# awkrail/svpc

Hardware: AMD Instinct MI355X
Metric: train steps/sec (vivt, batch=16, clip_seq=12) (higher is better)
Workload: dtype bf16x3; 1 GPU; MODEL_TYPE=vivt train step: N=16 videos/GPU x S=12 clips x Lv=100 frames x F=3072, Lt=22, D=768, H=12, L=6 (enc+step-enc+dec), V=951, A=384, E=10; dropout .1/.1/.4; fwd+bwd+allreduce+clip+BertAdam; mode=bf16x3, global_batch=16, parallelism=dp1, launch=hipGraph replay, gpus_requested=1

## Files before the change

include/svpc_hip.h:

```cpp
#ifndef SVPC_HIP_H
#define SVPC_HIP_H
#include <stddef.h>
#ifdef __cplusplus
extern "C" {
#endif

typedef struct ihipStream_t* svpc_stream_t;
typedef unsigned long long svpc_u64;

#define SVPC_ACT_NONE 0
#define SVPC_ACT_RELU 1
#define SVPC_ACT_GELU 2
#define SVPC_ACT_SIGMOID 3

const char* svpc_last_error(void);
int svpc_abi_version(void);

int svpc_ln_fwd(const float* x, const int* src_rows, const float* res, const float* gamma, const float* beta, float* y,
                float* mean, float* rstd, int R, int D, float eps, float p_pre, unsigned site_pre, float p_post,
                unsigned site_post, const svpc_u64* seed, const float* add1, int mod1, const float* add2, const int* idx2,
                svpc_stream_t stream);
int svpc_ln_fwd_t(const void* x, int x_dt, const int* src_rows, const void* res, const float* gamma, const float* beta, void* y,
                  int y_dt, float* mean, float* rstd, int R, int D, float eps, float p_pre, unsigned site_pre, float p_post,
                  unsigned site_post, const svpc_u64* seed, const float* add1, int mod1, const float* add2, const int* idx2,
// ... 196 lines not shown
                             svpc_stream_t stream);
int svpc_ptr_attn_gate_bwd_r(const float* dec, const float* proj, const float* bank, const int* step_ne, const float* pi, const float* dpi,
                             const float* pgen, const float* dpgen, const float* pgen_w, float* ddec, float* dproj, float* dbank,
                             float* wpart, int T, int lt, int e_max, int D, const int* row_off, const int* row_len, svpc_stream_t stream);
int svpc_ptr_mix_loss_fwd(const float* logits, const float* g, const float* pi, const int* labels, const int* row_c,
                          const int* row_vid, const int* csr_off, const int* csr_ent, const int* csr_id, const float* csr_w, float* P,
                          float* loss_rows, int R, int V, int c_max, int e_max, float smoothing, svpc_stream_t stream);
int svpc_ptr_mix_loss_bwd(const float* logits, const float* g, const float* pi, const int* labels, const int* row_c,
                          const int* row_vid, const int* csr_off, const int* csr_ent, const int* csr_id, const float* csr_w,
                          const float* P, const float* dP_ext, const float* dloss, float* dlogits, float* dg, float* dpi, int R, int V,
                          int c_max, int e_max, float smoothing, svpc_stream_t stream);
int svpc_ce_row_weights(const int* labels, const int* row_vid, int R, int n_vid, float* row_w, svpc_stream_t stream);
int svpc_ptr_mix_ce_fwd(const float* logits, const float* g, const float* pi, const int* labels, const int* row_c,
                        const int* row_vid, const int* csr_off, const int* csr_ent, const int* csr_id, const float* csr_w, float* P,
                        float* loss_rows, int R, int V, int c_max, int e_max, float smoothing, const float* row_w, svpc_stream_t stream);
int svpc_ptr_mix_ce_bwd(const float* logits, const float* g, const float* pi, const int* labels, const int* row_c,
                        const int* row_vid, const int* csr_off, const int* csr_ent, const int* csr_id, const float* csr_w,
                        const float* P, const float* dP_ext, const float* dloss, float* dlogits, float* dg, float* dpi, int R, int V,
                        int c_max, int e_max, float smoothing, const float* row_w, svpc_stream_t stream);

int svpc_gumbel_noise(float* out, size_t n, unsigned site, const svpc_u64* seed, svpc_stream_t stream);
int svpc_gumbel_fwd(const float* P, const float* noise, const int* row_c, const float* emb, float* bow, int* idx, float* stats, int R,
                    int c_max, int V, int W, float tau, svpc_stream_t stream);
int svpc_gumbel_bwd(const float* P, const float* noise, const int* row_c, const float* stats, const float* dy, float* dP, int R,
                    int c_max, int V, float tau, svpc_stream_t stream);
int svpc_gumbel_emb_grad(const float* dbow, const int* idx, const float* stats, float* demb, int R, int V, int W,
                         svpc_stream_t stream);

int svpc_rownorm_fwd(const float* a, float* y, int R, int C, int mode, svpc_stream_t stream);
int svpc_rownorm_bwd(const float* dy, const float* y, const float* a, float* da, int R, int C, int mode, svpc_stream_t stream);
int svpc_span_mean_fwd(const float* x, const int* starts, const int* lens, const float* w, const float* add, const int* add_idx,
                       float* out, int G, int D, svpc_stream_t stream);
int svpc_span_mean_bwd(const float* dout, const int* starts, const int* lens, const float* w, float* dx, int G, int D,
                       svpc_stream_t stream);
int svpc_scatter_add_rows(const float* dx, const int* idx, float* dtable, int R, int D, int pad_row, svpc_stream_t stream);
int svpc_bce_rows_fwd(const float* p, const float* y, const int* widths, float* out, int R, int C, svpc_stream_t stream);
int svpc_bce_rows_bwd(const float* dout, const float* p, const float* y, const int* widths, float* dp, int R, int C,
                      svpc_stream_t stream);
int svpc_asl_rows_fwd(const float* p, const float* y, const float* active, float* out, int R, int C, float gneg, float gpos,
                      float clip, float eps, svpc_stream_t stream);
int svpc_asl_rows_bwd(const float* dout, const float* p, const float* y, const float* active, float* dp, int R, int C, float gneg,
                      float gpos, float clip, float eps, svpc_stream_t stream);
int svpc_loss_tail_ws_floats(int n_cap, int R);
int svpc_loss_tail_fwd(const float* cap_rows, int n_cap, const float* e_p, const float* align, const int* widths, int R, int Ce,
                       const float* a_p, const float* act, int Ca, const float* r_e, const float* r_a, float lambda, float gneg,
                       float gpos, float clip, float eps, float* out5, float* workspace, int* counter, svpc_stream_t stream);
int svpc_loss_tail_bwd(const float* dout, int n_cap, const float* e_p, const float* align, const int* widths, int R, int Ce,
                       const float* a_p, const float* act, int Ca, const float* r_e, const float* r_a, float lambda, float gneg,
                       float gpos, float clip, float eps, float* d_cap, float* de_p, float* da_p, float* dr_e, float* dr_a,
                       svpc_stream_t stream);
int svpc_row_any_eq1(const float* x, float* out, int R, int C, svpc_stream_t stream);
int svpc_gather_cast_multi(const void* segments, int n, svpc_stream_t stream);
int svpc_gather_cast_multi_seed(const void* segments, int n, svpc_u64* bump_seed, svpc_stream_t stream);
int svpc_clamp_labels(const int* in, int* out, int n, int vocab, int unk, svpc_stream_t stream);
int svpc_lstm_cell_fwd(const float* gx, const float* gh, const float* c_prev, const float* h_prev, const float* active, float* h,
                       float* c, float* gates_act, int N, int D, svpc_stream_t stream);
int svpc_lstm_cell_bwd(const float* dh, const float* dc, const float* gates_act, const float* c_prev, const float* active,
                       float* dgates, float* dc_prev, float* dh_prev, int N, int D, svpc_stream_t stream);
int svpc_metric_argmax(const float* scores, int ld, int R, int C, const long long* labels, int ignore, double* counters,
                       svpc_stream_t stream);
int svpc_metric_f1(const float* prob, const float* gold, size_t n, double* counters, svpc_stream_t stream);
int svpc_gather_rows_f32(const float* src, const int* idx, float* dst, int rows, int width, svpc_stream_t stream);
int svpc_video_tokens(const int* n_valid, long long* ids, float* mask, int clips, int Lv, int L, int cls_id, int vid_id, int sep_id,
                      int pad_id, svpc_stream_t stream);
int svpc_lstm_cell_fwd_idx(const float* gx_all, const int* rows, const float* gh, const float* c_prev, const float* h_prev,
                           const float* active, float* h, float* c, float* gates_act, int N, int D, svpc_stream_t stream);
int svpc_lstm_cell_bwd_seq(const float* dh_out, const float* dh_rec, const float* dc, const float* gates_act, const float* c_prev,
                           const float* active, float* dgates, float* dc_prev, float* dh_prev, int N, int D, svpc_stream_t stream);
int svpc_lstm_pair_fwd(const float* const* gx, const int* const* rows, const float* const* gh, const float* const* c_prev,
                       const float* const* h_prev, const float* active, float* const* h, float* const* c, float* const* gates, int N, int D,
                       svpc_stream_t stream);
int svpc_lstm_pair_step_fwd(const float* const* h_prev, const float* const* c_prev, const float* const* w_hh, const float* const* gx,
                            const int* const* rows, const float* active, float* const* h, float* const* c, float* const* gates, int N,
                            int D, svpc_stream_t stream);
int svpc_lstm_pair_step_fwd_x3(const float* const* h_prev, const float* const* c_prev, const float* const* w_hh, const float* const* gx,
                               const int* const* rows, const float* active, float* const* h, float* const* c, float* const* gates, int N,
                               int D, svpc_stream_t stream);
int svpc_lstm_pair_bwd(const float* const* dh_out, const float* const* dh_rec, const float* const* dc, const float* const* gates,
                       const float* const* c_prev, const float* active, float* const* dgates, float* const* dc_prev,
                       float* const* dh_prev, int N, int D, svpc_stream_t stream);
int svpc_lstm_pair_bwd_parts(const float* const* dh_out, const float* const* dh_rec, const float* const* dh_parts, int n_parts,
                             const float* const* dc, const float* const* gates, const float* const* c_prev, const float* active,
                             float* const* dgates, float* const* dc_prev, float* const* dh_prev, int N, int D, svpc_stream_t stream);
int svpc_greedy_pick(const float* scores, int ld, const int* row_c, const int* row_x, int n_sent, int lt, int pos, int unk,
                     int* next_ext, int* next_model, svpc_stream_t stream);
int svpc_greedy_pick_append(const float* scores, int ld, const int* row_c, const int* row_x, int n_sent, int lt, int pos, int unk,
                            int* next_ext, int* next_model, int* text_out, int* ext_out, int ld_out, int col, svpc_stream_t stream);
int svpc_beam_step(const float* scores, int ld, const int* row_c, const int* row_x, int n_sent, int beam, int pos, int logits, int unk,
                   int eos, int pad, int slot_rows, float* cum, int* finished, const int* text_in, const int* ext_in, const int* rows_in,
                   int* text_out, int* ext_out, int* rows_out, int ld_tok, int* parent, int* next_ext, int* next_model, svpc_stream_t stream);
int svpc_beam_finalize(const float* cum, const int* ext, int ld_tok, int n_sent, int beam, int lt, int* best_ids, float* best_score,
                       svpc_stream_t stream);
int svpc_beam_step_ctl(const float* scores, int ld, const int* row_c, const int* row_x, int n_sent, int beam, int pos, int logits, int unk,
                       int eos, int pad, int slot_rows, float* cum, int* finished, const int* text_in, const int* ext_in, const int* rows_in,
                       int* text_out, int* ext_out, int* rows_out, int ld_tok, int* parent, int* next_ext, int* next_model, int min_len,
                       int ngram, const unsigned* excl, int excl_v, const double* lp, int* len, svpc_stream_t stream);
int svpc_beam_step_para(const float* scores, int ld, const int* row_c, const int* row_x, int n_sent, int beam, int pos, int logits, int unk,
                        int eos, int pad, int slot_rows, float* cum, int* finished, const int* text_in, const int* ext_in, const int* rows_in,
                        int* text_out, int* ext_out, int* rows_out, int ld_tok, int* parent, int* next_ext, int* next_model, int min_len,
                        int ngram, const unsigned* excl, int excl_v, const double* lp, int* len, const int* hist, const int* hist_desc,
                        int bos, svpc_stream_t stream);
int svpc_beam_step_groups(const float* scores, int ld, const int* row_c, const int* row_x, int n_sent, int beam, int pos, int logits, int unk,
                          int eos, int pad, int slot_rows, float* cum, int* finished, const int* text_in, const int* ext_in, const int* rows_in,
                          int* text_out, int* ext_out, int* rows_out, int ld_tok, int* parent, int* next_ext, int* next_model, int min_len,
                          int ngram, const unsigned* excl, int excl_v, const double* lp, int* len, int groups, const float* pen, float* aug,
                          svpc_stream_t stream);
int svpc_beam_finalize_nbest(const float* cum, const int* len, const double* lp, const int* ext, int ld_tok, int n_sent, int beam, int lt,
                             int n_best, int* best_ids, float* best_score, int* best_len, svpc_stream_t stream);
int svpc_sample_step(const float* scores, int ld, const int* row_c, const int* row_x, int n_rows, int max_c, int pos, int logits, int unk,
                     int eos, int pad, double temp, int topk, double topp, int min_len, const long long* seed, float* cum, int* finished,
                     int* len, int* text_out, int* ext_out, int ld_tok, int* next_ext, int* next_model, svpc_stream_t stream);
int svpc_sample_seed(const long long* src, long long* word, long long* used, svpc_stream_t stream);
int svpc_caption_clean(const void* ids, int ids64, long long ld, int row_stride, int row_pick, int n_rows, int lt, long long pad,
                       long long eos, long long ignore, int remove_dup, int* words, int* len, svpc_stream_t stream);
int svpc_caption_ngram_counts(const int* words, const int* len, const int* vid_off, int n_vid, int lt, int period, int comma, int vocab,
                              int* counts, unsigned* vocab_bits, svpc_stream_t stream);
int svpc_decode_metric_accum(const int* counts, int n_vid, double* acc, svpc_stream_t stream);
int svpc_caption_ingredients(const int* words, const int* len, int n_rows, int lt, const int* vid_off, const int* row_vs, int n_vid,
                             const unsigned* pred, int pred_ld, int n_pred, const unsigned* a_bits, int vocab, const int* vid,
                             const int* ing_tok, const int* tok_row, const unsigned* tok_oov, const int* eq_ids, const unsigned* oov_a,
                             const unsigned* gt_mask, const int* gt_len, const int* gx_off, const int* gx_ids, long long* masks, int* extra,
                             int* row_counts, int* vid_counts, unsigned long long* acc, svpc_stream_t stream);
int svpc_caption_tokens(const int* words, const int* len, const int* vid_off, int n_vid, int lt, int vocab, const int* voc_off,
                        const int* voc_tok, int n_voc_tok, const int* vid, const int* oov_off, int n_oov_off, const int* oov_tok,
                        int n_oov_tok, int* tokens, int* tok_len, svpc_stream_t stream);
int svpc_caption_score_counts(const int* tokens, const int* tok_len, int n_vid, const int* vid, const double* ref_norm,
                              const unsigned short* ref_tok, long long n_ref_tok, const unsigned long long* tab_key, const double* tab_idf,
                              int tab_cap, double log_docs, const double* gauss, int* counts, double* scores, long long* seen, int n_seen,
                              svpc_stream_t stream);
int svpc_caption_score_accum(const int* counts, const double* scores, int n_vid, unsigned long long* acc_i, double* acc_f,
                             svpc_stream_t stream);
int svpc_consensus_tokens(const int* words, const int* len, long long n_rows, const int* streams, int n_streams, int lt, int vocab,
                          const int* voc_off, const int* voc_tok, int n_voc_tok, const int* vid, int n_vid, const int* oov_off, int n_oov_off,
                          const int* oov_tok, int n_oov_tok, unsigned short* tokens, int* tok_len, svpc_stream_t stream);
int svpc_consensus_pair_scores(const unsigned short* tokens, const int* tok_len, int n_grp, int k, const unsigned long long* tab_key,
                               const double* tab_idf, int tab_cap, double log_docs, const double* gauss, double* out, double* work,
                               svpc_stream_t stream);
int svpc_consensus_pick(const double* pair, int n_grp, int k, int col, int posterior, const float* scores, const int* grp_off,
                        long long n_rows, const void* ids, int ids64, int lt, const long long* lengths, int* pick, double* expected,
                        long long* out_ids, long long* row_pick, float* out_scores, long long* out_len, svpc_stream_t stream);

int svpc_force_inputs(const void* ids, int ids_i64, int n_cap, int lt, int vocab, int unk, int eos, int pad, int ignore, int* model_ids,
                      float* mask, int* tgt, int* len, int* finished, svpc_stream_t stream);
int svpc_force_score(const float* scores, int ld, const int* row_c, int max_c, const int* tgt, const int* len, int n_cap, int lt, int logits,
                     int unk, int skip, float* step, int* rank, int* top, float* top_step, svpc_stream_t stream);
int svpc_force_finish(const int* tgt, const int* len, const int* row_c, int n_cap, int lt, int unk, int skip, float* step, int* rank,
                      int* top, float* top_step, float* cum, int* n_scored, svpc_stream_t stream);
int svpc_force_accum(const float* cum, const int* n_scored, const int* finished, const int* len, const int* rank, int n_cap, int lt,
                     double* acc, svpc_stream_t stream);

int svpc_seq_nll_fwd(const float* scores, int ld, const int* row_c, int max_c, const int* tgt, const int* len, const float* row_w,
                     int n_cap, int lt, int logits, int unk, float* step, float* cum, int* barred, float* loss, svpc_stream_t stream);
int svpc_seq_nll_bwd(const float* scores, int ld, const int* row_c, int max_c, const int* tgt, const int* len, const int* barred,
                     const float* row_w, const float* dl, int n_cap, int lt, int logits, int unk, float* dscores, int ld_out,
                     svpc_stream_t stream);
int svpc_scst_weights(const double* reward, const double* greedy, const int* row_vid, int n_vid, int k, int n_sent, int rule,
                      double* advantage, float* w, svpc_stream_t stream);

int svpc_rows_move(const void* src, int src_kind, int ld_src, int lo_src, const int* idx, void* dst, int dst_kind, int ld_dst, int lo_dst,
                   int R, int W, svpc_stream_t stream);
int svpc_scatter_add_rows_bf16(const float* rows, const int* idx, void* table, int ld_table, int R, int W, svpc_stream_t stream);
int svpc_pair_rows(float* a, const int* ia, float* b, const int* ib, float* out, float* out2, int R, int W, int mode, svpc_stream_t stream);
int svpc_add_cast_bf16(const void* a, const float* b, void* out, size_t n, svpc_stream_t stream);
int svpc_rows_expand(const float* src, const int* inv, float* out, int n_rows, int W, svpc_stream_t stream);
int svpc_add(const float* a, const float* b, float* c, size_t n, svpc_stream_t stream);
int svpc_sum_all(const float* x, size_t n, float* out, float scale, svpc_stream_t stream);
// ... 16 lines not shown
```

svpc_amd/csrc/gemm_l32.hip:

```cpp
#include "gemm_common.h"
#include <stdlib.h>

typedef __bf16 bf16x8 __attribute__((ext_vector_type(8)));
typedef const void __attribute__((address_space(1))) * l32_gptr;
typedef void __attribute__((address_space(3))) * l32_lptr;

constexpr int L32_BK = 32;
__device__ __attribute__((aligned(16))) const float l32_zeros[4] = {0.f, 0.f, 0.f, 0.f};

template <int N> __device__ __forceinline__ void l32_wait_vmcnt() { asm volatile("s_waitcnt vmcnt(%0)" ::"n"(N) : "memory"); }

template <int R, bool KC>
__device__ __forceinline__ const float* l32_src(const float* P, int ld, int m0, int rows, int k0, int j, int lane) {
    if (KC) {
        const int row = 8 * j + (lane >> 3), pos = lane & 7;
        const int c = pos ^ ((row >> 1) & 7);
        const int gr = min(m0 + row, rows - 1);
        return P + (size_t)gr * ld + k0 + 4 * c;
    } else {
        constexpr int CPR = R / 4;
        const int krow = j * (64 / CPR) + lane / CPR, c = lane % CPR;
        const int gm = min(m0 + 4 * c, rows - 4);
        return P + (size_t)(k0 + krow) * ld + gm;
    }
// ... 486 lines not shown
    skinny_partials<B_KC, NW, X3>(part, arow, brow, ldb, K);
    const u64 seed = epi.p_drop > 0.f ? epi.seed[0] : 0ull;
    const float inv_keep = epi.p_drop > 0.f ? 1.0f / (1.0f - epi.p_drop) : 1.0f;
    const int col = threadIdx.x & 31;
    constexpr int NE = 16 / NW;
    float vs[NE]; int rs[NE], cs[NE]; bool oks[NE];
#pragma unroll
    for (int i = 0; i < NE; ++i) {
        const int row = (threadIdx.x >> 5) + 2 * NW * i;
        const int e = (row & 3) + 4 * (row >> 3), l = col + 32 * ((row >> 2) & 1);
        float v = part[0][e][l];
#pragma unroll
        for (int w = 1; w < NW; ++w) v += part[w][e][l];
        vs[i] = v;
        oks[i] = row < ts && col < ts && m0 + row < M && n0 + col < N;
        rs[i] = min(m0 + row, M - 1); cs[i] = min(n0 + col, N - 1);
    }
    epilogue_store_n<NE>(vs, rs, cs, oks, C, ldc, epi, seed, inv_keep);
}
template <bool B_KC, bool X3 = false>
__global__ __launch_bounds__(256) void gemm_skinny_kernel(const float* __restrict__ A, int lda, const float* __restrict__ B, int ldb,
                                                          float* __restrict__ C, int ldc, int M, int N, int K, Epi epi, int tiles_n, int ts) {
    __shared__ float part[4][16][64];
    const int tm = blockIdx.x / tiles_n, tn = blockIdx.x - tm * tiles_n;
    skinny_tile<B_KC, 4, X3>(part, A, lda, B, ldb, C, ldc, M, N, K, epi, tm, tn, ts);
}
template <int NW, bool X3 = false, bool B_KC = true>
__global__ __launch_bounds__(64 * NW) void gemm_group_skinny_kernel(GemmGroupArgs g) {
    __shared__ float part[NW][16][64];
    int pi = 0;
    while (pi + 1 < g.n && (int)blockIdx.x >= g.p[pi + 1].tile0) ++pi;
    const GemmProb& q = g.p[pi];
    const int tile = blockIdx.x - q.tile0;
    const int tm = tile / q.tiles_n, tn = tile - tm * q.tiles_n;
    Epi epi{nullptr, ACT_NONE, 0.f, 0u, nullptr, g.accumulate, nullptr};
    skinny_tile<B_KC, NW, X3>(part, q.A, q.lda, q.B, q.ldb, q.C, q.ldc, q.M, q.N, q.K, epi, tm, tn);
}

struct LstmStep {
    const float* h_prev[2]; const float* c_prev[2]; const float* w_hh[2]; const float* gx[2]; const int* rows[2]; const float* active;
    float* h[2]; float* c[2]; float* gates[2]; int N, D;
};
template <bool X3>
__global__ __launch_bounds__(256) void lstm_pair_step_fwd_kernel(LstmStep a) {
    __shared__ float part[4][16][64];
    const int z = blockIdx.y, u0 = blockIdx.x * 8, m0 = blockIdx.z * 32;
    const int lane = threadIdx.x & 63, r = lane & 31, hh = lane >> 5;
    const int N = a.N, D = a.D;
    const float* arow = a.h_prev[z] + (size_t)min(m0 + r, N - 1) * D + 8 * hh;
    const float* brow = a.w_hh[z] + (size_t)((r >> 3) * D + u0 + (r & 7)) * D + 8 * hh;
    const int row = threadIdx.x >> 3, j = threadIdx.x & 7, n = m0 + row;
    const int nc = min(n, N - 1), dpre = u0 + j;
    const float* gxp = a.gx[z] + (size_t)a.rows[z][nc] * 4 * D + dpre;
    const float gx0 = gxp[0], gx1 = gxp[D], gx2 = gxp[2 * D], gx3 = gxp[3 * D];
    const float cp_pre = a.c_prev[z][(size_t)nc * D + dpre], hp_pre = a.h_prev[z][(size_t)nc * D + dpre], act_pre = a.active[nc];
    skinny_partials<true, 4, X3>(part, arow, brow, D, D);
    if (n >= N) return;
    float gsum[4];
    const int e = (row & 3) + 4 * (row >> 3), lb = 32 * ((row >> 2) & 1);
#pragma unroll
    for (int g = 0; g < 4; ++g) {
        const int l = g * 8 + j + lb;
        float v = part[0][e][l];
#pragma unroll
        for (int w = 1; w < 4; ++w) v += part[w][e][l];
        gsum[g] = v;
    }
    const int d = u0 + j;
    const size_t i = (size_t)n * D + d, g0 = (size_t)n * 4 * D + d;
    const float gi = sigmoidf_(gx0 + gsum[0]);
    const float gf = sigmoidf_(gx1 + gsum[1]);
    const float gg = tanhf(gx2 + gsum[2]);
    const float go = sigmoidf_(gx3 + gsum[3]);
    float* ga = a.gates[z];
    ga[g0] = gi; ga[g0 + D] = gf; ga[g0 + 2 * D] = gg; ga[g0 + 3 * D] = go;
    const float cp = cp_pre;
    const float cn = gf * cp + gi * gg;
    const float hn = go * tanhf(cn);
    const float act = act_pre;
    a.c[z][i] = act * cn + (1.f - act) * cp;
    a.h[z][i] = act * hn + (1.f - act) * hp_pre;
}

extern "C" {

static int lstm_pair_step_fwd_x(const float* const* h_prev, const float* const* c_prev, const float* const* w_hh, const float* const* gx,
                                const int* const* rows, const float* active, float* const* h, float* const* c, float* const* gates, int N,
                                int D, int x3, hipStream_t stream) {
    if (N == 0) return 0;
    SVPC_REQUIRE(D % 16 == 0 && D >= 16, "lstm_pair_step_fwd: hidden size must be a multiple of 16");
    LstmStep a{};
    for (int z = 0; z < 2; ++z) {
        SVPC_REQUIRE(((((uintptr_t)h_prev[z]) | ((uintptr_t)w_hh[z])) & 15) == 0, "lstm_pair_step_fwd: 16-byte aligned state / weight rows");
        a.h_prev[z] = h_prev[z]; a.c_prev[z] = c_prev[z]; a.w_hh[z] = w_hh[z]; a.gx[z] = gx[z]; a.rows[z] = rows[z];
        a.h[z] = h[z]; a.c[z] = c[z]; a.gates[z] = gates[z];
    }
    a.active = active; a.N = N; a.D = D;
    if (x3) hipLaunchKernelGGL(lstm_pair_step_fwd_kernel<true>, dim3(D / 8, 2, ceil_div(N, 32)), dim3(256), 0, stream, a);
    else hipLaunchKernelGGL(lstm_pair_step_fwd_kernel<false>, dim3(D / 8, 2, ceil_div(N, 32)), dim3(256), 0, stream, a);
    return svpc_check_launch("lstm_pair_step_fwd");
}
int svpc_lstm_pair_step_fwd(const float* const* h_prev, const float* const* c_prev, const float* const* w_hh, const float* const* gx,
                            const int* const* rows, const float* active, float* const* h, float* const* c, float* const* gates, int N,
                            int D, hipStream_t stream) {
    return lstm_pair_step_fwd_x(h_prev, c_prev, w_hh, gx, rows, active, h, c, gates, N, D, 0, stream);
}
int svpc_lstm_pair_step_fwd_x3(const float* const* h_prev, const float* const* c_prev, const float* const* w_hh, const float* const* gx,
                               const int* const* rows, const float* active, float* const* h, float* const* c, float* const* gates, int N,
                               int D, hipStream_t stream) {
    return lstm_pair_step_fwd_x(h_prev, c_prev, w_hh, gx, rows, active, h, c, gates, N, D, 1, stream);
}

int svpc_gemm_l32_supported(int a_kc, int b_kc, int lda, int ldb, int M, int N, int K) {
    if (M <= 0 || N <= 0 || K <= 0 || lda % 4 != 0 || ldb % 4 != 0) return 0;
    if (K % L32_BK != 0 && !(a_kc && b_kc && K % 4 == 0 && K > L32_BK)) return 0;
    if (!a_kc && (M % 4 != 0)) return 0;
    if (!b_kc && (N % 4 != 0)) return 0;
    return 1;
}

int svpc_gemm_l32_preferred(int a_kc, int b_kc, int lda, int ldb, int M, int N, int K) {
    if (!svpc_gemm_l32_supported(a_kc, b_kc, lda, ldb, M, N, K)) return 0;
    const int t128 = ceil_div(M, 128) * ceil_div(N, 128), t64 = ceil_div(M, 64) * ceil_div(N, 64);
    static int env_w = -1;
    if (env_w < 0) { const char* e = getenv("SVPC_L32_WAVESPLIT"); env_w = e ? atoi(e) : 1; }
    if (K % L32_BK != 0) return (t128 <= 300) ? 1 : 0;
    if (env_w && t64 <= 256 && K >= 4 * L32_BK && t64 * 4 >= 32) return 1;
    return (t128 <= 300 && K < 2048) ? 1 : 0;
}

struct HostWgradProblem { const float* dz; const float* x; float* dw; float* db; int n_out, n_in, rows, ld_dz, ld_x, ld_dw; };

int svpc_gemm_group_wgrad_max(void) { return GROUP_MAX; }

static int gemm_group_x(const void* problems, int n, int a_kc, int b_kc, int accumulate, int x3, hipStream_t stream) {
    if (n == 0) return 0;
    SVPC_REQUIRE(n > 0 && n <= GEMM_GROUP_MAX, "gemm_group: 1..32 problems per launch");
    const HostGemmProblem* hp = reinterpret_cast<const HostGemmProblem*>(problems);
    GemmGroupArgs g{};
    g.n = n; g.accumulate = accumulate;
    int tiles = 0;
    static int env_skinny = -1;
    if (env_skinny < 0) { const char* e = getenv("SVPC_L32_SKINNY"); env_skinny = e ? atoi(e) : 1; }
    bool skinny = env_skinny && a_kc;
    if (!b_kc && x3) skinny = false;
    int kmax = 0;
    for (int i = 0; i < n; ++i) {
        if (hp[i].M > 256 || hp[i].N < 32 || (hp[i].K & 15) || (hp[i].lda & 3) || (hp[i].ldb & 3)) skinny = false;
        if (hp[i].K > kmax) kmax = hp[i].K;
    }
    const int T = skinny ? 32 : 64;
    for (int i = 0; i < n; ++i) {
        const HostGemmProblem& h = hp[i];
        SVPC_REQUIRE(svpc_gemm_l32_supported(a_kc, b_kc, h.lda, h.ldb, h.M, h.N, h.K) && h.K % L32_BK == 0 && ((((uintptr_t)h.A) | ((uintptr_t)h.B)) & 15) == 0,
                     "gemm_group: needs K % 32 == 0 and 16-byte aligned fp32 rows");
        GemmProb& q = g.p[i];
        q.A = h.A; q.B = h.B; q.C = h.C; q.M = h.M; q.N = h.N; q.K = h.K; q.lda = h.lda; q.ldb = h.ldb; q.ldc = h.ldc;
        q.tile0 = tiles; q.tiles_n = ceil_div(h.N, T);
        tiles += ceil_div(h.M, T) * q.tiles_n;
    }
    if (skinny && !b_kc) {
        if (kmax >= 1536) hipLaunchKernelGGL((gemm_group_skinny_kernel<8, false, false>), dim3(tiles), dim3(512), 0, stream, g);
        else hipLaunchKernelGGL((gemm_group_skinny_kernel<4, false, false>), dim3(tiles), dim3(256), 0, stream, g);
        return svpc_check_launch("gemm_group_skinny");
    }
    if (skinny) {
        if (x3) {
// ... 175 lines not shown
```

svpc_amd/ops.py:

```python
from __future__ import annotations

import ctypes
import math
import numbers
import os
import struct

import torch
from torch.autograd import Function as _TorchFunction

from . import _lib
from .ops_common import ACT_GELU, ACT_NONE, ACT_RELU, ACT_SIGMOID, FIdx, Idx, SeqInfo, as_idx

_WS = {}
_WS_BYTES = 256 << 20


_DEV_IDX = [None]


def _stream():
    i = _DEV_IDX[0]
    if i is None or not _FAST_STREAM:
        return torch.cuda.current_stream().cuda_stream
# ... 1942 lines not shown
    return _LstmCell.apply(gx, gh, c_prev, h_prev, active)


class _LstmSeq(Function):

    @staticmethod
    def forward(ctx, gx_all, w_hh, rows_t, active_t, pick, wgrad):
        _need_gpu(gx_all)
        gx_all, w = _c(gx_all), _c(w_hh)
        S, N = len(rows_t), rows_t[0].numel()
        D = w.shape[1]
        dev = gx_all.device
        h_all = torch.empty(S + 1, N, D, dtype=torch.float32, device=dev)
        c_all = torch.empty(S + 1, N, D, dtype=torch.float32, device=dev)
        h_all[0].zero_(); c_all[0].zero_()
        gates = torch.empty(S, N, 4 * D, dtype=torch.float32, device=dev)
        gh = torch.empty(N, 4 * D, dtype=torch.float32, device=dev)
        for t in range(S):
            _gemm(h_all[t], D, 1, w, D, 1, gh, N, 4 * D, D)
            _lib.call("lstm_cell_fwd_idx", _p(gx_all), _p(rows_t[t]), _p(gh), _p(c_all[t]), _p(h_all[t]), _p(active_t[t]),
                      _p(h_all[t + 1]), _p(c_all[t + 1]), _p(gates[t]), N, D, _stream())
        out = torch.index_select(h_all[1:].reshape(S * N, D), 0, pick)
        ctx.save_for_backward(gates, c_all, h_all, w, pick)
        ctx.lists = (rows_t, active_t)
        ctx.direct = wgrad
        ctx.cfg = (S, N, D, gx_all.shape[0])
        return out

    @staticmethod
    def backward(ctx, dout):
        gates, c_all, h_all, w, pick = ctx.saved_tensors
        rows_t, active_t = ctx.lists
        S, N, D, T = ctx.cfg
        dev = dout.device
        dhs = torch.zeros(S * N, D, dtype=torch.float32, device=dev)
        dhs.index_copy_(0, pick.long() if pick.dtype != torch.int64 else pick, _c(dout))
        dhs = dhs.view(S, N, D)
        dG = torch.empty(S, N, 4 * D, dtype=torch.float32, device=dev)
        dh = torch.zeros(N, D, dtype=torch.float32, device=dev)
        dc = torch.zeros(N, D, dtype=torch.float32, device=dev)
        dh2, dc2 = torch.empty_like(dh), torch.empty_like(dc)
        wt = w.t().contiguous()
        for t in range(S - 1, -1, -1):
            _lib.call("lstm_cell_bwd_seq", _p(dhs[t]), _p(dh), _p(dc), _p(gates[t]), _p(c_all[t]), _p(active_t[t]), _p(dG[t]), _p(dc2),
                      _p(dh2), N, D, _stream())
            _gemm(dG[t], 4 * D, 1, wt, 4 * D, 1, dh2, N, D, 4 * D, accumulate=1)
            dh, dh2 = dh2, dh
            dc, dc2 = dc2, dc
        dG2, hp = dG.view(S * N, 4 * D), h_all[:S].reshape(S * N, D)
        wgrad = ctx.direct
        dw = None
        if wgrad is not None or ctx.needs_input_grad[1]:
            acc = 1 if wgrad is not None else 0
            dw = wgrad if wgrad is not None else torch.empty_like(w)
            with _side_of(wgrad, dG2, hp):
                _gemm(dG2, 4 * D, 0, hp, D, 0, dw, 4 * D, D, S * N, accumulate=acc)
            if wgrad is not None:
                _ready(wgrad, "w")
                dw = None
        dgx = torch.index_select(dG2, 0, pick) if ctx.needs_input_grad[0] else None
        return dgx, dw, None, None, None, None


class _GemmProblem(ctypes.Structure):
    _fields_ = [("A", ctypes.c_void_p), ("B", ctypes.c_void_p), ("C", ctypes.c_void_p), ("M", ctypes.c_int), ("N", ctypes.c_int),
                ("K", ctypes.c_int), ("lda", ctypes.c_int), ("ldb", ctypes.c_int), ("ldc", ctypes.c_int)]


def _gemm_pair(As, Bs, Cs, M, N, K, accumulate=0, x3=False):
    probs = (_GemmProblem * 2)()
    for z in range(2):
        probs[z] = _GemmProblem(As[z].data_ptr(), Bs[z].data_ptr(), Cs[z].data_ptr(), M, N, K, As[z].stride(0), Bs[z].stride(0),
                                Cs[z].stride(0))
    _lib.call("gemm_group_x3" if x3 else "gemm_group", ctypes.addressof(probs), 2, 1, 1, accumulate, _stream())


def _ptr2(a, b):
    arr = (ctypes.c_void_p * 2)(a.data_ptr(), b.data_ptr())
    return ctypes.addressof(arr), arr


LSTM_DGRAD_PARTS = int(os.environ.get("SVPC_LSTM_DGRAD_PARTS", "4"))
LSTM_FUSED_STEP = os.environ.get("SVPC_LSTM_FUSED_STEP", "1") != "0"


class _BiLstmSeq(Function):

    @staticmethod
    def forward(ctx, gx_f, gx_b, w_f, w_b, rows_f, rows_b, active_t, pick_f, pick_b, wgrad_f, wgrad_b, summed=False):
        _need_gpu(gx_f)
        ctx.summed = bool(summed)
        gx = [_c(gx_f), _c(gx_b)]
        w = [_c(w_f), _c(w_b)]
        rows = [rows_f, rows_b]
        S, N = len(rows_f), rows_f[0].numel()
        D = w[0].shape[1]
        dev = gx_f.device
        mk = lambda *sh: torch.empty(*sh, dtype=torch.float32, device=dev)
        state = mk(2, 2, S + 1, N, D)
        state[:, :, 0].zero_()
        h_all, c_all = [state[0, 0], state[1, 0]], [state[0, 1], state[1, 1]]
        gates = [mk(S, N, 4 * D) for _ in range(2)]
        gh = [mk(N, 4 * D) for _ in range(2)]
        st = _stream()
        fused = LSTM_FUSED_STEP and D % 16 == 0 and (w[0].data_ptr() | w[1].data_ptr()) % 16 == 0
        pw = _ptr2(w[0], w[1])
        pgx = _ptr2(gx[0], gx[1])
        for t in range(S):
            args = [pgx, _ptr2(rows[0][t], rows[1][t]), _ptr2(gh[0], gh[1]), _ptr2(c_all[0][t], c_all[1][t]),
                    _ptr2(h_all[0][t], h_all[1][t]), None, _ptr2(h_all[0][t + 1], h_all[1][t + 1]),
                    _ptr2(c_all[0][t + 1], c_all[1][t + 1]), _ptr2(gates[0][t], gates[1][t])]
            if fused:
                _lib.call("lstm_pair_step_fwd_x3" if is_x3() else "lstm_pair_step_fwd", args[4][0], args[3][0], pw[0], args[0][0],
                          args[1][0], _p(active_t[t]), args[6][0], args[7][0], args[8][0], N, D, st)
                continue
            _gemm_pair([h_all[0][t], h_all[1][t]], w, gh, N, 4 * D, D, x3=is_x3())
            _lib.call("lstm_pair_fwd", args[0][0], args[1][0], args[2][0], args[3][0], args[4][0], _p(active_t[t]), args[6][0],
                      args[7][0], args[8][0], N, D, st)
        ctx.save_for_backward(gates[0], gates[1], c_all[0], c_all[1], h_all[0], h_all[1], w[0], w[1], pick_f, pick_b)
        ctx.lists = active_t
        ctx.direct = (wgrad_f, wgrad_b)
        ctx.cfg = (S, N, D)
        pair_ok = (D % 4 == 0 and pick_f.dtype == torch.int32 and pick_b.dtype == torch.int32 and pick_f.numel() == pick_b.numel())
        ctx.pair_ok = pair_ok
        if summed and pair_ok:
            out = mk(pick_f.numel(), D)
            _lib.call("pair_rows", _p(h_all[0][1:]), _p(pick_f), _p(h_all[1][1:]), _p(pick_b), _p(out), None, pick_f.numel(), D, 0, st)
            return out
        outs = [torch.index_select(h_all[z][1:].reshape(S * N, D), 0, pk) for z, pk in enumerate((pick_f, pick_b))]
        if summed:
            return outs[0] + outs[1]
        return outs[0], outs[1]

    @staticmethod
    def backward(ctx, dout_f, dout_b=None):
        if ctx.summed:
            dout_b = dout_f
        g0, g1, c0, c1, h0, h1, w0, w1, pick_f, pick_b = ctx.saved_tensors
        gates, c_all, h_all, w, picks = [g0, g1], [c0, c1], [h0, h1], [w0, w1], [pick_f, pick_b]
        active_t = ctx.lists
        S, N, D = ctx.cfg
        dev = g0.device
        mk = lambda *sh: torch.empty(*sh, dtype=torch.float32, device=dev)
        zeros = torch.zeros(2 * S * N + 4 * N, D, dtype=torch.float32, device=dev)
        dhs = []
        if ctx.summed and ctx.pair_ok and dout_f is not None:
            _lib.call("pair_rows", _p(zeros), _p(picks[0]), _p(zeros[S * N:]), _p(picks[1]), _p(_c(dout_f)), None, picks[0].numel(), D, 1,
                      _stream())
            dhs = [zeros[:S * N].view(S, N, D), zeros[S * N:2 * S * N].view(S, N, D)]
        else:
            for z, d in enumerate((dout_f, dout_b)):
                t_ = zeros[z * S * N:(z + 1) * S * N]
                if d is not None:
                    t_.index_copy_(0, picks[z].long(), _c(d))
                dhs.append(t_.view(S, N, D))
        dG = [mk(S, N, 4 * D) for _ in range(2)]
        tail = zeros[2 * S * N:].view(4, N, D)
        dh = [tail[0], tail[1]]
        dc = [tail[2], tail[3]]
        dh2, dc2 = [mk(N, D) for _ in range(2)], [mk(N, D) for _ in range(2)]
        st = _stream()
        P = LSTM_DGRAD_PARTS if (4 * D) % (32 * LSTM_DGRAD_PARTS) == 0 else 1
        Kp = 4 * D // P
        slabs = [mk(P, N, D) for _ in range(2)] if P > 1 else None
        have_parts = False
        for t in range(S - 1, -1, -1):
            a = [_ptr2(dhs[0][t], dhs[1][t]), _ptr2(dh[0], dh[1]), _ptr2(dc[0], dc[1]), _ptr2(gates[0][t], gates[1][t]),
                 _ptr2(c_all[0][t], c_all[1][t]), None, _ptr2(dG[0][t], dG[1][t]), _ptr2(dc2[0], dc2[1]), _ptr2(dh2[0], dh2[1])]
            if P > 1:
                sp = _ptr2(slabs[0], slabs[1])
                _lib.call("lstm_pair_bwd_parts", a[0][0], a[1][0], sp[0] if have_parts else None, P if have_parts else 0, a[2][0], a[3][0],
                          a[4][0], _p(active_t[t]), a[6][0], a[7][0], a[8][0], N, D, st)
                if t > 0:
                    probs = (_GemmProblem * (2 * P))()
                    for z in range(2):
                        for k in range(P):
                            probs[z * P + k] = _GemmProblem(dG[z][t].data_ptr() + 4 * k * Kp, w[z].data_ptr() + 4 * k * Kp * D,
                                                            slabs[z][k].data_ptr(), N, D, Kp, 4 * D, D, D)
                    _lib.call("gemm_group", ctypes.addressof(probs), 2 * P, 1, 0, 0, st)
                    have_parts = True
            else:
                _lib.call("lstm_pair_bwd", a[0][0], a[1][0], a[2][0], a[3][0], a[4][0], _p(active_t[t]), a[6][0], a[7][0], a[8][0], N, D, st)
                wt = [w[z].t().contiguous() for z in range(2)] if t == S - 1 else wt
                _gemm_pair([dG[0][t], dG[1][t]], wt, dh2, N, D, 4 * D, accumulate=1)
            dh, dh2 = dh2, dh
            dc, dc2 = dc2, dc
        dws, dgx = [None, None], [None, None]
        for z in range(2):
            dG2, hp = dG[z].view(S * N, 4 * D), h_all[z][:S].reshape(S * N, D)
            wgrad = ctx.direct[z]
            if wgrad is not None or ctx.needs_input_grad[2 + z]:
                if not (wgrad is not None and defer_wgrad(dG2, hp, wgrad, None)):
                    acc = 1 if wgrad is not None else 0
                    dw = wgrad if wgrad is not None else torch.empty_like(w[z])
                    _gemm(dG2, 4 * D, 0, hp, D, 0, dw, 4 * D, D, S * N, accumulate=acc)
                    if wgrad is not None:
                        _ready(wgrad, "w")
                    else:
                        dws[z] = dw
            if ctx.needs_input_grad[z] and not (ctx.pair_ok and ctx.needs_input_grad[0] and ctx.needs_input_grad[1]):
                dgx[z] = torch.index_select(dG2, 0, picks[z])
        if ctx.pair_ok and ctx.needs_input_grad[0] and ctx.needs_input_grad[1]:
            R_ = picks[0].numel()
            dgx = [mk(R_, 4 * D), mk(R_, 4 * D)]
            _lib.call("pair_rows", _p(dG[0]), _p(picks[0]), _p(dG[1]), _p(picks[1]), _p(dgx[0]), _p(dgx[1]), R_, 4 * D, 2, _stream())
        return dgx[0], dgx[1], dws[0], dws[1], None, None, None, None, None, None, None, None


def bilstm_sequences(gx_f, gx_b, w_f, w_b, rows_f, rows_b, active_t, pick_f, pick_b, summed=False):
    if _fast() and gx_f.is_cuda and not BWD_EXACT:
        return _BiLstmSeq.apply(gx_f, gx_b, w_f, w_b, rows_f, rows_b, active_t, pick_f, pick_b, _direct(w_f), _direct(w_b), summed)
    of, ob = lstm_sequence(gx_f, w_f, rows_f, active_t, pick_f), lstm_sequence(gx_b, w_b, rows_b, active_t, pick_b)
    return add(of, ob) if summed else (of, ob)


def lstm_sequence(gx_all, w_hh, rows_t, active_t, pick):
    return _LstmSeq.apply(gx_all, w_hh, rows_t, active_t, pick, _direct(w_hh))


class _BceRows(Function):
    @staticmethod
    def forward(ctx, p, y, widths):
        _need_gpu(p)
        p, y = _c(p), _c(y)
        R, C = p.shape
        w = widths.dev(p.device)
        out = torch.empty(R, dtype=torch.float32, device=p.device)
        _lib.call("bce_rows_fwd", _p(p), _p(y), _p(w), _p(out), R, C, _stream())
        ctx.save_for_backward(p, y, w)
        return out

    @staticmethod
    def backward(ctx, dout):
        p, y, w = ctx.saved_tensors
        dp = torch.empty_like(p)
        _lib.call("bce_rows_bwd", _p(_c(dout)), _p(p), _p(y), _p(w), _p(dp), p.shape[0], p.shape[1], _stream())
        return dp, None, None


def bce_rows(p, y, widths):
    return _BceRows.apply(p, y, as_idx(widths))


class _AslRows(Function):
    @staticmethod
    def forward(ctx, p, y, active, gneg, gpos, clip, eps):
        _need_gpu(p)
        p, y = _c(p), _c(y)
        R, C = p.shape
        out = torch.empty(R, dtype=torch.float32, device=p.device)
        _lib.call("asl_rows_fwd", _p(p), _p(y), _p(active), _p(out), R, C, gneg, gpos, clip, eps, _stream())
        ctx.save_for_backward(p, y, active)
# ... 928 lines not shown
```

Baseline: 90.24 steps/s (one step = 16 clip-sequences per GPU; whole-job aggregate).

## Fuse LSTM backward recurrent dgrad GEMM into per-step pointwise kernel with bf16 MFMA

Adds a fused kernel that runs the recurrent dh GEMM (previous step's dgates times W_hh) with bf16 MFMA on pre-swizzled fragments, then applies the LSTM cell backward pointwise math in the same launch. This replaces the separate pair_bwd_parts kernel plus the grouped split-K gemm at each timestep. W_hh is converted once per call into a bf16 fragment layout, and dgates are also written as bf16 fragments for the next step. The recurrent gradient is now computed in bf16 instead of the earlier precision, which risks a small accuracy change, and one kernel per step does the reduction across 8 waves through shared memory.

Measured after the change: 91.07 steps/s (one step = 16 clip-sequences per GPU; whole-job aggregate), median of 6. Within noise of the previous version (+0.9%).

```diff
diff --git a/include/svpc_hip.h b/include/svpc_hip.h
--- a/include/svpc_hip.h
+++ b/include/svpc_hip.h
@@ -302,6 +302,11 @@
 int svpc_lstm_pair_bwd_parts(const float* const* dh_out, const float* const* dh_rec, const float* const* dh_parts, int n_parts,
                              const float* const* dc, const float* const* gates, const float* const* c_prev, const float* active,
                              float* const* dgates, float* const* dc_prev, float* const* dh_prev, int N, int D, svpc_stream_t stream);
+int svpc_lstm_pair_step_bwd(const float* const* dh_out, const float* const* dh_pass, const float* const* dc, const float* const* gates,
+                            const float* const* c_prev, const float* active, const void* const* dg_next_frag,
+                            const void* const* w_hh_frag, float* const* dgates, void* const* dgates_frag, float* const* dc_prev,
+                            float* const* dh_prev, int N, int D, svpc_stream_t stream);
+int svpc_lstm_whh_frag(const float* const* w_hh, void* const* out, int D, svpc_stream_t stream);
 int svpc_greedy_pick(const float* scores, int ld, const int* row_c, const int* row_x, int n_sent, int lt, int pos, int unk,
                      int* next_ext, int* next_model, svpc_stream_t stream);
 int svpc_greedy_pick_append(const float* scores, int ld, const int* row_c, const int* row_x, int n_sent, int lt, int pos, int unk,
diff --git a/svpc_amd/csrc/gemm_l32.hip b/svpc_amd/csrc/gemm_l32.hip
--- a/svpc_amd/csrc/gemm_l32.hip
+++ b/svpc_amd/csrc/gemm_l32.hip
@@ -592,7 +592,119 @@
     a.h[z][i] = act * hn + (1.f - act) * hp_pre;
 }
 
+typedef float l32_floatx4 __attribute__((ext_vector_type(4)));
+typedef __bf16 l32_bf16x4 __attribute__((ext_vector_type(4)));
+struct LstmStepBwd {
+    const float* dh_out[2]; const float* dh_pass[2]; const float* dc[2]; const float* gates[2]; const float* c_prev[2]; const float* active;
+    const __bf16* dg_next[2]; const __bf16* wf[2];
+    float* dgates[2]; __bf16* dg_bf[2]; float* dc_prev[2]; float* dh_prev[2]; int N, D;
+};
+__global__ __launch_bounds__(512) void lstm_pair_step_bwd_kernel(LstmStepBwd a) {
+    constexpr int BATCH = 12;
+    __shared__ float part[8][4][64];
+    const int z = blockIdx.y, u0 = blockIdx.x * 16, m0 = blockIdx.z * 16;
+    const int lane = threadIdx.x & 63, wave = __builtin_amdgcn_readfirstlane(threadIdx.x >> 6);
+    const int N = a.N, D = a.D, K = 4 * D;
+    const int nsteps = K >> 5;
+    const int pair = threadIdx.x & 255;
+    const int row = pair >> 4, j = pair & 15, n = m0 + row;
+    const int nc = min(n, N - 1), d = u0 + j;
+    const size_t i = (size_t)nc * D + d, g0 = (size_t)nc * K + d;
+    const float* ga = a.gates[z];
+    const float gi = ga[g0], gf = ga[g0 + D], gg = ga[g0 + 2 * D], go = ga[g0 + 3 * D];
+    const float dho = a.dh_out[z][i], dhp = a.dh_pass[z][i], dci = a.dc[z][i], cp = a.c_prev[z][i], act = a.active[nc];
+    l32_floatx4 acc = {0.f, 0.f, 0.f, 0.f};
+    const __bf16* dgn = a.dg_next[z];
+    if (dgn != nullptr) {
+        const __bf16* af = dgn + ((size_t)blockIdx.z * nsteps * 64 + lane) * 8;
+        const __bf16* bf = a.wf[z] + ((size_t)blockIdx.x * nsteps * 64 + lane) * 8;
+        auto batch = [&](int s0) {
+            bf16x8 av[BATCH], bv[BATCH];
+#pragma unroll
+            for (int u = 0; u < BATCH; ++u) {
+                const int s = min(s0 + 8 * u, nsteps - 1);
+                av[u] = *reinterpret_cast<const bf16x8*>(af + (size_t)s * 512);
+                bv[u] = *reinterpret_cast<const bf16x8*>(bf + (size_t)s * 512);
+            }
+#pragma unroll
+            for (int u = 0; u < BATCH; ++u)
+                if (s0 + 8 * u < nsteps) acc = __builtin_amdgcn_mfma_f32_16x16x32_bf16(av[u], bv[u], acc, 0, 0, 0);
+        };
+        if (wave < nsteps) batch(wave);
+        for (int s0 = wave + 8 * BATCH; s0 < nsteps; s0 += 8 * BATCH) batch(s0);
+    }
+#pragma unroll
+    for (int e = 0; e < 4; ++e) part[wave][e][lane] = acc[e];
+    __syncthreads();
+    if (threadIdx.x >= 256 || n >= N) return;
+    const int e = row & 3, l = j + 16 * (row >> 2);
+    float rec = part[0][e][l];
+#pragma unroll
+    for (int w = 1; w < 8; ++w) rec += part[w][e][l];
+    const float dht = (dho + dhp) + rec;
+    const float dhn = act * dht, dcn_in = act * dci;
+    const float cn = gf * cp + gi * gg;
+    const float tc = tanhf(cn);
+    const float dcn = dcn_in + dhn * go * (1.f - tc * tc);
+    const float dv[4] = {dcn * gg * gi * (1.f - gi), dcn * cp * gf * (1.f - gf), dcn * gi * (1.f - gg * gg), dhn * tc * go * (1.f - go)};
+    float* dg = a.dgates[z];
+    __bf16* db = a.dg_bf[z] + (size_t)blockIdx.z * nsteps * 512;
+#pragma unroll
+    for (int g = 0; g < 4; ++g) {
+        const int k = g * D + d;
+        dg[g0 + (size_t)g * D] = dv[g];
+        db[((size_t)(k >> 5) * 64 + 16 * ((k >> 3) & 3) + row) * 8 + (k & 7)] = (__bf16)dv[g];
+    }
+    a.dc_prev[z][i] = dcn * gf + (1.f - act) * dci;
+    a.dh_prev[z][i] = (1.f - act) * dht;
+}
+__global__ __launch_bounds__(256) void lstm_whh_frag_kernel(const float* w0, const float* w1, __bf16* o0, __bf16* o1, int D) {
+    __shared__ float tile[32][33];
+    const float* __restrict__ w = blockIdx.z ? w1 : w0;
+    __bf16* __restrict__ o = blockIdx.z ? o1 : o0;
+    const int k0 = blockIdx.x * 32, u0 = blockIdx.y * 32, nsteps = D >> 3;
+    const int tx = threadIdx.x & 31, ty = threadIdx.x >> 5;
+#pragma unroll
+    for (int r = ty; r < 32; r += 8) tile[r][tx] = u0 + tx < D ? w[(size_t)(k0 + r) * D + u0 + tx] : 0.f;
+    __syncthreads();
+    const int ut = threadIdx.x >> 7, l = (threadIdx.x >> 1) & 63, half = threadIdx.x & 1;
+    if (u0 + 16 * ut >= D) return;
+    const int kg = l >> 4, c = l & 15;
+    l32_bf16x4 v;
+#pragma unroll
+    for (int q = 0; q < 4; ++q) v[q] = (__bf16)tile[8 * kg + 4 * half + q][16 * ut + c];
+    *reinterpret_cast<l32_bf16x4*>(o + (((size_t)(2 * blockIdx.y + ut) * nsteps + blockIdx.x) * 64 + l) * 8 + 4 * half) = v;
+}
+
 extern "C" {
+
+int svpc_lstm_pair_step_bwd(const float* const* dh_out, const float* const* dh_pass, const float* const* dc, const float* const* gates,
+                            const float* const* c_prev, const float* active, const void* const* dg_next_frag,
+                            const void* const* w_hh_frag, float* const* dgates, void* const* dgates_frag, float* const* dc_prev,
+                            float* const* dh_prev, int N, int D, hipStream_t stream) {
+    if (N == 0) return 0;
+    SVPC_REQUIRE(D % 16 == 0 && D >= 16, "lstm_pair_step_bwd: hidden size must be a multiple of 16");
+    LstmStepBwd a{};
+    for (int z = 0; z < 2; ++z) {
+        a.dh_out[z] = dh_out[z]; a.dh_pass[z] = dh_pass[z]; a.dc[z] = dc[z]; a.gates[z] = gates[z]; a.c_prev[z] = c_prev[z];
+        a.dg_next[z] = dg_next_frag ? static_cast<const __bf16*>(dg_next_frag[z]) : nullptr;
+        a.wf[z] = static_cast<const __bf16*>(w_hh_frag[z]);
+        SVPC_REQUIRE(((((uintptr_t)a.dg_next[z]) | ((uintptr_t)a.wf[z])) & 15) == 0 && a.wf[z] != nullptr && dgates_frag[z] != nullptr,
+                     "lstm_pair_step_bwd: 16-byte aligned fragment buffers");
+        a.dgates[z] = dgates[z]; a.dg_bf[z] = static_cast<__bf16*>(dgates_frag[z]); a.dc_prev[z] = dc_prev[z]; a.dh_prev[z] = dh_prev[z];
+    }
+    SVPC_REQUIRE((a.dg_next[0] == nullptr) == (a.dg_next[1] == nullptr), "lstm_pair_step_bwd: dg_next of both directions or of neither");
+    a.active = active; a.N = N; a.D = D;
+    hipLaunchKernelGGL(lstm_pair_step_bwd_kernel, dim3(D / 16, 2, ceil_div(N, 16)), dim3(512), 0, stream, a);
+    return svpc_check_launch("lstm_pair_step_bwd");
+}
+int svpc_lstm_whh_frag(const float* const* w_hh, void* const* out, int D, hipStream_t stream) {
+    SVPC_REQUIRE(D % 16 == 0 && D >= 16, "lstm_whh_frag: hidden size must be a multiple of 16");
+    SVPC_REQUIRE(((((uintptr_t)out[0]) | ((uintptr_t)out[1])) & 15) == 0, "lstm_whh_frag: 16-byte aligned output");
+    hipLaunchKernelGGL(lstm_whh_frag_kernel, dim3(4 * D / 32, ceil_div(D, 32), 2), dim3(256), 0, stream, w_hh[0], w_hh[1],
+                       static_cast<__bf16*>(out[0]), static_cast<__bf16*>(out[1]), D);
+    return svpc_check_launch("lstm_whh_frag");
+}
 
 static int lstm_pair_step_fwd_x(const float* const* h_prev, const float* const* c_prev, const float* const* w_hh, const float* const* gx,
                                 const int* const* rows, const float* active, float* const* h, float* const* c, float* const* gates, int N,
diff --git a/svpc_amd/ops.py b/svpc_amd/ops.py
--- a/svpc_amd/ops.py
+++ b/svpc_amd/ops.py
@@ -2048,6 +2048,7 @@
 
 LSTM_DGRAD_PARTS = int(os.environ.get("SVPC_LSTM_DGRAD_PARTS", "4"))
 LSTM_FUSED_STEP = os.environ.get("SVPC_LSTM_FUSED_STEP", "1") != "0"
+LSTM_FUSED_STEP_BWD = os.environ.get("SVPC_LSTM_FUSED_STEP_BWD", "1") != "0"
 
 
 class _BiLstmSeq(Function):
@@ -2128,12 +2129,23 @@
         st = _stream()
         P = LSTM_DGRAD_PARTS if (4 * D) % (32 * LSTM_DGRAD_PARTS) == 0 else 1
         Kp = 4 * D // P
-        slabs = [mk(P, N, D) for _ in range(2)] if P > 1 else None
         have_parts = False
+        fused = LSTM_FUSED_STEP_BWD and D % 16 == 0
+        slabs = [mk(P, N, D) for _ in range(2)] if P > 1 and not fused else None
+        if fused:
+            wt = torch.empty(2, D, 4 * D, dtype=torch.bfloat16, device=dev)
+            dGb = torch.empty(2, S, 16 * ((N + 15) // 16), 4 * D, dtype=torch.bfloat16, device=dev)
+            pwt, pw = _ptr2(wt[0], wt[1]), _ptr2(w[0], w[1])
+            _lib.call("lstm_whh_frag", pw[0], pwt[0], D, st)
         for t in range(S - 1, -1, -1):
             a = [_ptr2(dhs[0][t], dhs[1][t]), _ptr2(dh[0], dh[1]), _ptr2(dc[0], dc[1]), _ptr2(gates[0][t], gates[1][t]),
                  _ptr2(c_all[0][t], c_all[1][t]), None, _ptr2(dG[0][t], dG[1][t]), _ptr2(dc2[0], dc2[1]), _ptr2(dh2[0], dh2[1])]
-            if P > 1:
+            if fused:
+                nxt = _ptr2(dGb[0][t + 1], dGb[1][t + 1]) if t < S - 1 else (None, None)
+                cur = _ptr2(dGb[0][t], dGb[1][t])
+                _lib.call("lstm_pair_step_bwd", a[0][0], a[1][0], a[2][0], a[3][0], a[4][0], _p(active_t[t]), nxt[0], pwt[0], a[6][0],
+                          cur[0], a[7][0], a[8][0], N, D, st)
+            elif P > 1:
                 sp = _ptr2(slabs[0], slabs[1])
                 _lib.call("lstm_pair_bwd_parts", a[0][0], a[1][0], sp[0] if have_parts else None, P if have_parts else 0, a[2][0], a[3][0],
                           a[4][0], _p(active_t[t]), a[6][0], a[7][0], a[8][0], N, D, st)
```
